# FindoraNetwork/ark-bulletproofs

Hardware: AMD Instinct MI355X
Metric: r1cs_constraints_proved_per_sec (+ r1cs_batch_verifies_per_sec under "verify") (higher is better)
Workload: dtype u32x9 (256-bit modular integers, radix 2^29)

## Files before the change

### ark_bulletproofs_amd/csrc/arkbp.hip

```cpp
#include <hip/hip_runtime.h>
#include <sys/prctl.h>
#include <time.h>
#include <rccl/rccl.h>
#include <dlfcn.h>
#include <mutex>
#include <cmath>
#include <cstdio>
#include <cstring>
#include <algorithm>
#include <deque>
#include <array>
#include <functional>
#include <map>
#include <memory>
#include <set>
#include <string>
#include <tuple>
#include <unordered_map>
#include <vector>
#include "../../include/arkbp.h"
#include <atomic>
#include <chrono>
#include "host_proto.hpp"
#include "prove_steps.hpp"
// ... 596 lines not shown
    done = !over;
    return BP_OK;
}
template <class C> static bool msm_glv_route(const bp_ctx* ctx, const BaseSegs& segs, size_t n, bool sharded, int w_hi) {
    if constexpr (!C::HAS_GLV) { (void)ctx; (void)segs; (void)n; (void)sharded; (void)w_hi; return false; }
    else {
        static const bool no_glv = getenv("ARKBP_MSM_NOGLV") != nullptr, no_fs0 = getenv("ARKBP_MSM_NOFS") != nullptr;
        return !no_glv && !no_fs0 && !sharded && w_hi < 0 && ctx->shard_world == 1 && !segs.fixed_c4 && msm_glv_sizes(msm_knobs(ctx), n);
    }
}

template <class C, class Finish>
static int msm_tree_back(bp_ctx* ctx, const BaseSegs& segs, const u32* entries, int mode, const SlotPlan& sp, const MsmPlan& pl, const u32* tot, int nl, int chl,
                         bool special, int spl, u32 b_gen, u32 top_nb, bool wave, int& K, bool& deep, Finish&& finish) {
    hipStream_t st = ctx->stream;
    const int TB = 256;
    const size_t Bp1 = (size_t)pl.B + 1;
    u32* lvl = ctx->lvl_off.as<u32>();
    K = 1;
    { u64 cap = (u64)1 << chl; while (cap < tot[MSM_NLMAX]) { cap <<= chl; K++; } }
    if (special && K < spl + 1) K = spl + 1;
    deep = K >= nl;
    if (deep) return BP_OK;
    BPCHK(ctx->lvA.ensure((size_t)tot[1] * 96));
    if (K >= 2) BPCHK(ctx->lvB.ensure((size_t)tot[2] * 96));
    if (wave && !special) {
        ScopedK acc(ctx, BP_K_MSM_ACCUM);
        hipLaunchKernelGGL(k_msm_accum_wave<C>, dim3((pl.B + 3) / 4), dim3(256), 0, st, segs, entries, lvl, lvl + Bp1 * K, ctx->lvA.as<u32>(), pl.B, mode, sp, (u32)pl.NB,
                           ctx->boff.as<u32>());
        acc.stop();
        finish(ctx->lvA.as<u32>(), lvl + Bp1 * K);
        return BP_OK;
    }
    {
        ScopedK acc(ctx, BP_K_MSM_ACCUM);
        hipLaunchKernelGGL(k_msm_accum<C>, dim3((tot[1] + TB - 1) / TB), dim3(TB), 0, st, segs, entries, lvl, lvl + Bp1, ctx->lvA.as<u32>(), pl.B, tot[1], mode, sp, (u32)pl.NB,
                           ctx->boff.as<u32>(), chl);
    }
    u32* cur = ctx->lvA.as<u32>();
    u32* nxt = ctx->lvB.as<u32>();
    ScopedK agg(ctx, BP_K_MSM_AGG);
    for (int k = 2; k <= K; k++) {
        hipLaunchKernelGGL(k_msm_reduce<C>, dim3((tot[k] + TB - 1) / TB), dim3(TB), 0, st, cur, lvl + Bp1 * (k - 1), lvl + Bp1 * k, nxt, pl.B, tot[k], chl,
                           (k == spl + 1 && special) ? b_gen : pl.B);
        if (k == spl + 1 && special)
            hipLaunchKernelGGL(k_msm_reduce_special<C>, dim3(top_nb), dim3(256), 0, st, cur, lvl + Bp1 * spl, lvl + Bp1 * (spl + 1), nxt, b_gen, pl.B);
        u32* t = cur; cur = nxt; nxt = t;
    }
    finish(cur, lvl + Bp1 * K);
    return BP_OK;
}

template <class C> static int msm_run(bp_ctx* ctx, const BaseSegs& segs, const u32* d_scalars_one, size_t n, int scalars_mont, J4& result,
                                      int w_lo = 0, int w_hi = -1 ,
                                      int shard_mode = -1 ,
                                      const ScalSegs* sseg = nullptr ,
                                      bool no_fixed_shape = false ) {
    ScalSegs d_scalars; memset(&d_scalars, 0, sizeof d_scalars);
    if (sseg) d_scalars = *sseg; else { d_scalars.nseg = 1; d_scalars.ptr[0] = d_scalars_one; d_scalars.start[0] = 0; d_scalars.start[1] = (u32)n; }
    typedef host::Grp<C> G;
    result = G::inf();
    if (n == 0) return BP_OK;
    if (n >= (1u << 31)) { g_err = "msm: n too large"; return BP_E_ARG; }
    hipStream_t st = ctx->stream;
    const MsmKnobs kn = msm_knobs(ctx);
    MsmPlan pl = msm_plan(n, C::Fr::BITS, kn);
    const bool sharded = w_hi < 0 && ctx->shard_world > 1 && shard_mode != 0;
    if (sharded && shard_mode != 2) {
        const int base = pl.W / ctx->shard_world, rem = pl.W % ctx->shard_world, r = ctx->shard_rank;
// ... 3599 lines not shown
```

### ark_bulletproofs_amd/csrc/ec.cuh

```cuda
#pragma once
#include "fp29.cuh"

namespace arkbp {

struct Aff {
    Fe x, y;
};
struct Jac {
    Fe X, Y, Z;
};

ARKBP_HD bool aff_is_inf(const Aff& p) { return fe_is_zero_exact(p.x) && fe_is_zero_exact(p.y); }
ARKBP_HD bool jac_is_inf(const Jac& p) { return fe_is_zero_exact(p.Z); }
template <class C> ARKBP_HD Jac jac_inf() {
    Jac r;
    r.X = fe_one<typename C::Fq>();
    r.Y = fe_one<typename C::Fq>();
    r.Z = fe_zero<typename C::Fq>();
    return r;
}
template <class C> ARKBP_HD Jac jac_from_aff(const Aff& p) {
    if (aff_is_inf(p)) return jac_inf<C>();
    Jac r;
    r.X = p.x;
// ... 104 lines not shown
template <class C> ARKBP_HD Jac jac_add(const Jac& p, const Jac& q) {
    typedef typename C::Fq F;
    if (jac_is_inf(q)) return p;
    if (jac_is_inf(p)) return q;
    Fe Z1Z1 = fe_sqr<F>(p.Z), Z2Z2 = fe_sqr<F>(q.Z);
    Fe U1 = fe_mul<F>(p.X, Z2Z2), U2 = fe_mul<F>(q.X, Z1Z1);
    Fe S1 = fe_mul<F>(p.Y, fe_mul<F>(q.Z, Z2Z2)), S2 = fe_mul<F>(q.Y, fe_mul<F>(p.Z, Z1Z1));
    Fe H = fe_sub<F, 2>(U2, U1);
    Fe r = fe_sub<F, 2>(S2, S1);
    if (fe_is_zero_mod<F>(H)) {
        if (fe_is_zero_mod<F>(r)) return jac_dbl<C>(p);
        return jac_inf<C>();
    }
    Fe HH = fe_sqr<F>(H);
    Fe HHH = fe_mul<F>(H, HH);
    Fe V = fe_mul<F>(U1, HH);
    Jac o;
    o.X = fe_wred<F>(fe_sub<F, 4>(fe_sqr<F>(r), fe_add(HHH, fe_dbl(V))));
    o.Y = fe_mul2<F>(r, fe_sub<F, 4>(V, o.X), fe_neg<F, 2>(S1), HHH);
    o.Z = fe_mul<F>(fe_mul<F>(p.Z, q.Z), H);
    return o;
}

template <class C> ARKBP_HD Aff jac_to_aff_with_zinv(const Jac& p, const Fe& zinv) {
    typedef typename C::Fq F;
    Aff r;
    if (jac_is_inf(p)) {
        r.x = fe_zero<F>();
        r.y = fe_zero<F>();
        return r;
    }
    Fe zi2 = fe_sqr<F>(zinv);
    r.x = fe_canon<F>(fe_mul<F>(p.X, zi2));
    r.y = fe_canon<F>(fe_mul<F>(p.Y, fe_mul<F>(zi2, zinv)));
    return r;
}
template <class C> ARKBP_HD Aff jac_to_aff(const Jac& p) {
    return jac_to_aff_with_zinv<C>(p, fe_inv<typename C::Fq>(p.Z));
}

template <class F> ARKBP_DEV_NOINLINE bool fe_sqrt(Fe& out, const Fe& a_in) {
    const Fe a = fe_wred<F>(a_in);
    if (fe_is_zero_mod<F>(a)) { out = fe_zero<F>(); return true; }
    const Fe a2 = fe_sqr<F>(a), a3 = fe_mul<F>(a2, a);
    Fe w = fe_one<F>();
#pragma unroll 1
// ... 90 lines not shown
```

### ark_bulletproofs_amd/csrc/ipa.cuh

```cuda
#pragma once
#include "msm.cuh"

namespace arkbp {

template <class F> __global__ void k_scalars_import(const u32* __restrict__ in, u32* __restrict__ out, u32 n) {
    const u32 i = blockIdx.x * blockDim.x + threadIdx.x;
    if (i >= n) return;
    u32 w[8];
    load_words8(w, in + (size_t)i * 8);
    store_fe_dev<F>(out + (size_t)i * 8, fe_load_ark<F>(w));
}
template <class F> __global__ void k_scalars_export(const u32* __restrict__ in, u32* __restrict__ out, u32 n) {
    const u32 i = blockIdx.x * blockDim.x + threadIdx.x;
    if (i >= n) return;
    u32 w[8];
    fe_store_ark<F>(w, load_fe_dev<F>(in + (size_t)i * 8));
    store_words8(out + (size_t)i * 8, w);
}

static constexpr int IMPORT_MAX = 5;
struct ImportList {
    u32* dst[IMPORT_MAX];
    u32 cnt[IMPORT_MAX];
    int nseg;
// ... 484 lines not shown
            const Aff cur = load_aff_dev(row + ((size_t)(e - 1) * n + i) * 16);
            if (!jac_equals_aff<C>(jac_madd<C>(jac_from_aff<C>(prev), base), cur)) wrong++;
            prev = cur;
        }
        expect = jac_dbl<C>(jac_from_aff<C>(prev));
    }
    if (wrong) atomicAdd(bad, (unsigned long long)wrong);
}
template <class C> __global__ void __launch_bounds__(256)
k_fb_rows_check(const u32* __restrict__ gens, const u32* __restrict__ T, u32 n, size_t row_points, u32 R, unsigned long long* __restrict__ bad) {
    const u32 i = blockIdx.x * blockDim.x + threadIdx.x;
    if (i >= n) return;
    u32 wrong = 0;
    Jac expect = jac_from_aff<C>(load_aff_dev(gens + (size_t)i * 16));
#pragma unroll 1
    for (u32 r = 0; r < R; r++) {
        const Aff cur = load_aff_dev(T + ((size_t)r * row_points + i) * 16);
        if (!jac_equals_aff<C>(expect, cur)) wrong++;
        expect = jac_dbl<C>(jac_dbl<C>(jac_dbl<C>(jac_dbl<C>(jac_from_aff<C>(cur)))));
    }
    if (wrong) atomicAdd(bad, (unsigned long long)wrong);
}

template <class C> __device__ __forceinline__ Jac ftab_step(Jac acc, const u32* __restrict__ T, u32 n_tab, u32 E, u32 gi, u32 j, u32 e1, u32 e2, bool neg1, bool neg2) {
    typedef typename C::Fq F;
#pragma unroll 1
    for (int h = 0; h < (C::HAS_GLV ? 2 : 1); h++) {
        const u32 e = h ? e2 : e1;
        if (!e) continue;
        const u32* src = T + (((size_t)j * E + (e - 1)) * n_tab + gi) * 16;
        const bool neg = h ? neg2 : neg1;
        Aff P = load_aff_dev(src);
        if constexpr (C::HAS_GLV) { if (h && !aff_is_inf(P)) P.x = fe_mul<F>(P.x, fe_const<F, C::BETA29>()); }
        bool rare;
        Jac nxt = jac_madd_fast<C>(acc, aff_cneg_lazy<C>(P, neg), rare);
        if (__builtin_expect(rare, 0)) {
            Aff Q = load_aff_dev(src);
            if constexpr (C::HAS_GLV) { if (h && !aff_is_inf(Q)) Q.x = fe_mul<F>(Q.x, fe_const<F, C::BETA29>()); }
            nxt = jac_madd<C>(acc, aff_cneg_lazy<C>(Q, neg));
        }
        acc = nxt;
    }
    return acc;
}
template <class C> __global__ void __launch_bounds__(256) __attribute__((amdgpu_waves_per_eu(3)))
k_ipa_fold_tab(const u32* __restrict__ TG, const u32* __restrict__ TH, u32 n_tab, u32 E, u32* __restrict__ G, u32* __restrict__ H, u32 n, FtabDigits dG,
               FtabDigits dH, int which, u32 g_first, u32 g_stride, u32* __restrict__ jac_ws,
               const u32* __restrict__ Gin ,
               const u32* __restrict__ Hin) {
    typedef typename C::Fq F;
    const u32 t = blockIdx.x * blockDim.x + threadIdx.x;
    if (t >= (which == 3 ? 2 * n : n)) return;
    const bool isH = which == 2 || (which == 3 && t >= n);
    const u32 i = (which == 3 && isH) ? t - n : t;
    u32* V = isH ? H : G;
    const u32* T = isH ? TH : TG;
    const u32 gi = g_first + i * g_stride;
    Jac acc = jac_inf<C>();
    const u32 nwin = isH ? dH.nwin : dG.nwin;
#pragma unroll 1
    for (u32 j = 0; j < nwin; j++) {
        const u32 e1 = isH ? dH.e1[j] : dG.e1[j], e2 = isH ? dH.e2[j] : dG.e2[j];
        acc = ftab_step<C>(acc, T, n_tab, E, gi, j, e1, e2, (((isH ? dH.neg1 : dG.neg1) >> j) & 1ull) != 0, (((isH ? dH.neg2 : dG.neg2) >> j) & 1ull) != 0);
    }
    const u32* Vin = isH ? (Hin ? Hin : H) : (Gin ? Gin : G);
    acc = jac_madd<C>(acc, load_aff_dev(Vin + (size_t)(n + i) * 16));
    fold_emit<C>(V, i, t, acc, jac_ws);
}

struct FtabDigits3 {
    FtabDigits d[3];
};
template <class C> __global__ void __launch_bounds__(256) __attribute__((amdgpu_waves_per_eu(3)))
k_ipa_fold_tab2(const u32* __restrict__ TG, const u32* __restrict__ TH, u32 n_tab, u32 E, u32* __restrict__ G, u32* __restrict__ H, u32 m, FtabDigits3 dG,
                FtabDigits3 dH, u32* __restrict__ jac_ws, const u32* __restrict__ Gin, const u32* __restrict__ Hin,
                u32 g_first , u32 g_stride) {
    typedef typename C::Fq F;
    const u32 t = blockIdx.x * blockDim.x + threadIdx.x;
    if (t >= 2 * m) return;
    const bool isH = t >= m;
    const u32 i = isH ? t - m : t;
    const u32 n = 2 * m;
    const u32* T = isH ? TH : TG;
    Jac acc = jac_inf<C>();
#pragma unroll 1
    for (u32 mu = 0; mu < 3; mu++) {
        const u32 gi = g_first + (mu == 0 ? m + i : mu == 1 ? n + i : i) * g_stride;
        const u32 nwin = isH ? dH.d[mu].nwin : dG.d[mu].nwin;
        const unsigned long long neg1 = isH ? dH.d[mu].neg1 : dG.d[mu].neg1, neg2 = isH ? dH.d[mu].neg2 : dG.d[mu].neg2;
#pragma unroll 1
        for (u32 j = 0; j < nwin; j++) {
            const u32 e1 = isH ? dH.d[mu].e1[j] : dG.d[mu].e1[j], e2 = isH ? dH.d[mu].e2[j] : dG.d[mu].e2[j];
            acc = ftab_step<C>(acc, T, n_tab, E, gi, j, e1, e2, ((neg1 >> j) & 1ull) != 0, ((neg2 >> j) & 1ull) != 0);
        }
    }
    acc = jac_madd<C>(acc, load_aff_dev((isH ? Hin : Gin) + (size_t)(n + m + i) * 16));
    fold_emit<C>(isH ? H : G, i, t, acc, jac_ws);
}

}
```

### ark_bulletproofs_amd/csrc/msm.cuh

```cuda
#pragma once
#include "ec.cuh"
#include "fe_io.cuh"
#include "ecq.cuh"
#include "glv.cuh"
#include "msm_plan.hpp"

namespace arkbp {

static constexpr int MSM_MAXSEG = 6;

struct BaseSegs {
    const u32* ptr[MSM_MAXSEG];
    u32 start[MSM_MAXSEG + 1];
    int nseg;
    u32 fixed_c4;
    u32 tbits;
    u64 row_words[MSM_MAXSEG];
    u32 glv;
    u32 stride[MSM_MAXSEG];
};
__device__ __forceinline__ const u32* seg_base_ptr(const BaseSegs& s, u32 idx) {
    u32 w = 0;
    if (s.glv) idx >>= 1;
    if (s.fixed_c4) { w = idx >> s.tbits; idx &= (1u << s.tbits) - 1u; }
// ... 34 lines not shown
    const uint4* q = reinterpret_cast<const uint4*>(p);
    Raw16 r;
    r.a = q[0]; r.b = q[1]; r.c = q[2]; r.d = q[3];
    return r;
}
__device__ __forceinline__ Aff aff_from_raw(const Raw16& r) {
    const u32 w[16] = {r.a.x, r.a.y, r.a.z, r.a.w, r.b.x, r.b.y, r.b.z, r.b.w, r.c.x, r.c.y, r.c.z, r.c.w, r.d.x, r.d.y, r.d.z, r.d.w};
    return aff_load_dev(w);
}
template <class C> __device__ __forceinline__ void store_jac_ws(u32* p, const Jac& j) {
    typedef typename C::Fq F;
    u32 w[8];
    fe_pack(w, fe_canon<F>(j.X)); store_words8(p, w);
    fe_pack(w, fe_canon<F>(j.Y)); store_words8(p + 8, w);
    fe_pack(w, fe_canon<F>(j.Z)); store_words8(p + 16, w);
}
__device__ __forceinline__ Jac load_jac_ws(const u32* p) {
    u32 w[8];
    Jac j;
    load_words8(w, p); j.X = fe_unpack(w);
    load_words8(w, p + 8); j.Y = fe_unpack(w);
    load_words8(w, p + 16); j.Z = fe_unpack(w);
    return j;
}

__device__ __forceinline__ int msm_digit(const u32 k[8], int w, int c, u32& carry) {
    const int bit = w * c;
    const int wi = bit >> 5, bo = bit & 31;
    u64 x = 0;
    if (wi < 8) x = k[wi];
    if (wi + 1 < 8) x |= (u64)k[wi + 1] << 32;
    u32 d = ((u32)(x >> bo) & ((1u << c) - 1)) + carry;
    carry = d > (1u << (c - 1)) ? 1u : 0u;
    return (int)d - (int)(carry << c);
}

__device__ __forceinline__ void load_words12(u32 w[12], const u32* p) {
    const uint4* q = reinterpret_cast<const uint4*>(p);
    const uint4 a = q[0], b = q[1], c = q[2];
    w[0] = a.x; w[1] = a.y; w[2] = a.z; w[3] = a.w; w[4] = b.x; w[5] = b.y; w[6] = b.z; w[7] = b.w; w[8] = c.x; w[9] = c.y; w[10] = c.z; w[11] = c.w;
}
__device__ __forceinline__ void store_words12(u32* p, const u32 w[12]) {
    uint4* q = reinterpret_cast<uint4*>(p);
    q[0] = make_uint4(w[0], w[1], w[2], w[3]); q[1] = make_uint4(w[4], w[5], w[6], w[7]); q[2] = make_uint4(w[8], w[9], w[10], w[11]);
}
__device__ __forceinline__ void glv_half(const u32 g[12], int h, u32 k[8], bool& neg) {
// ... 359 lines not shown
#pragma unroll
    for (int j = 0; j < 8; j++) k[j] = 0;
    if (live) load_words8(k, canon + (size_t)i * 8);
    u32 carry = 0;
    for (int w = 0; w < pl.W; w++) {
        const int d = msm_digit(k, w, pl.c, carry);
        const bool valid = live && d != 0 && w >= pl.w_lo && w < pl.w_hi;
        const u32 pos = wave_count(cursor, (u32)w * pl.NB + (u32)(d < 0 ? -d : d) - 1, valid);
        if (valid) entries[pos] = (i << 1) | (d < 0 ? 1u : 0u);
    }
}

__device__ __forceinline__ u32 find_bucket(const u32* __restrict__ off, u32 B, u32 j) {
    u32 lo = 0, hi = B;
    while (hi - lo > 1) {
        u32 mid = (lo + hi) >> 1;
        if (off[mid] <= j) lo = mid; else hi = mid;
    }
    return lo;
}

template <class C> __global__ void __launch_bounds__(256)
k_msm_accum(BaseSegs segs, const u32* __restrict__ entries, const u32* __restrict__ off0, const u32* __restrict__ off1, u32* __restrict__ out,
            u32 B, u32 nchunks, int slotted, SlotPlan sp, u32 NB, const u32* __restrict__ boff, int chl) {
    const u32 j = blockIdx.x * blockDim.x + threadIdx.x;
    if (j >= nchunks) return;
    const u32 b = find_bucket(off1, B, j);
    u32 beg, end;
    const u32 r = j - off1[b], k = off1[b + 1] - off1[b];
    u32 s0, cnt;
    if (slotted == 2) {
        s0 = boff[b]; cnt = off0[b + 1] - off0[b];
    } else if (slotted) {
        const u32 w = b / NB, v = b - w * NB;
        s0 = sp.base[w] + v * sp.cap[w]; cnt = off0[b + 1] - off0[b];
    } else {
        s0 = off0[b]; cnt = off0[b + 1] - off0[b];
    }
    const u32 per = k > 1 ? (cnt + k - 1) / k : (1u << chl);
    beg = s0 + min(r * per, cnt);
    end = min(beg + per, s0 + cnt);
    Jac acc = jac_inf<C>();
    if (beg < end) {
        u32 ent = entries[beg];
        u32 ent_n = beg + 1 < end ? entries[beg + 1] : 0u;
        Raw16 raw = load_raw16(seg_base_ptr(segs, ent >> 1));
        for (u32 e = beg; e < end; e++) {
            Raw16 raw_n = raw;
            u32 ent_nn = 0;
            if (e + 1 < end) raw_n = load_raw16(seg_base_ptr(segs, ent_n >> 1));
            if (e + 2 < end) ent_nn = entries[e + 2];
            const Aff p = aff_from_raw(raw);
            if (e == beg) {
                acc = jac_from_aff<C>(aff_cneg_lazy<C>(p, ent & 1));
                acc.Y = fe_wred<typename C::Fq>(acc.Y);
            } else {
                bool rare;
                Jac nxt = jac_madd_fast<C>(acc, aff_cneg_lazy<C>(p, ent & 1), rare);
                if (__builtin_expect(rare, 0)) nxt = jac_madd<C>(acc, aff_cneg_lazy<C>(load_aff_dev(seg_base_ptr(segs, ent >> 1)), ent & 1));
                acc = nxt;
            }
            ent = ent_n; ent_n = ent_nn;
            raw = raw_n;
        }
    }
    store_jac_ws<C>(out + (size_t)j * 24, acc);
}

template <class C> __global__ void __launch_bounds__(256)
k_msm_accum_wave(BaseSegs segs, const u32* __restrict__ entries, const u32* __restrict__ off0, const u32* __restrict__ off_last, u32* __restrict__ out, u32 B,
                 int slotted, SlotPlan sp, u32 NB, const u32* __restrict__ boff) {
    __shared__ u32 sh[4][64 * 27];
    const u32 wv = threadIdx.x >> 6, lane = threadIdx.x & 63;
    const u32 b = blockIdx.x * 4 + wv;
    if (b >= B) return;
    const u32 cnt = off0[b + 1] - off0[b];
    if (!cnt) return;
    u32 beg;
    if (slotted == 2) beg = boff[b];
    else if (slotted) { const u32 w = b / NB, v = b - w * NB; beg = sp.base[w] + v * sp.cap[w]; }
    else beg = off0[b];
    Jac acc = jac_inf<C>();
    for (u32 e = lane; e < cnt; e += 64) {
        const u32 ent = entries[beg + e];
        acc = jac_madd<C>(acc, aff_cneg_lazy<C>(load_aff_dev(seg_base_ptr(segs, ent >> 1)), ent & 1));
    }
    u32* s = sh[wv];
    for (u32 stride = 32; stride >= 1; stride >>= 1) {
        if (lane >= stride && lane < 2 * stride) {
#pragma unroll
            for (int i = 0; i < 9; i++) { s[i * 64 + lane] = acc.X.l[i]; s[(9 + i) * 64 + lane] = acc.Y.l[i]; s[(18 + i) * 64 + lane] = acc.Z.l[i]; }
        }
        __builtin_amdgcn_wave_barrier();
        __threadfence_block();
        if (lane < stride) {
            Jac o;
#pragma unroll
            for (int i = 0; i < 9; i++) { o.X.l[i] = s[i * 64 + lane + stride]; o.Y.l[i] = s[(9 + i) * 64 + lane + stride]; o.Z.l[i] = s[(18 + i) * 64 + lane + stride]; }
            acc = jac_add<C>(acc, o);
        }
        __builtin_amdgcn_wave_barrier();
        __threadfence_block();
    }
    if (lane == 0) store_jac_ws<C>(out + (size_t)off_last[b] * 24, acc);
}

template <class C> __global__ void __launch_bounds__(256)
k_msm_reduce(const u32* __restrict__ in, const u32* __restrict__ off_prev, const u32* __restrict__ off_cur, u32* __restrict__ out, u32 B,
             u32 nchunks, int chl, u32 skip_from ) {
    const u32 j = blockIdx.x * blockDim.x + threadIdx.x;
    if (j >= nchunks) return;
    const u32 b = find_bucket(off_cur, B, j);
    if (b >= skip_from) return;
    const u32 beg = off_prev[b] + ((j - off_cur[b]) << chl);
    const u32 end = min(beg + (1u << chl), off_prev[b + 1]);
    Jac acc = load_jac_ws(in + (size_t)beg * 24);
    for (u32 e = beg + 1; e < end; e++) acc = jac_add<C>(acc, load_jac_ws(in + (size_t)e * 24));
    store_jac_ws<C>(out + (size_t)j * 24, acc);
}

template <class C, u32 NT = 256> __device__ __forceinline__ Jac block_sum_jac(Jac acc, u32* __restrict__ sh ) {
    const u32 tid = threadIdx.x;
    for (u32 stride = NT / 2; stride >= 1; stride >>= 1) {
        if (tid >= stride && tid < 2 * stride) {
#pragma unroll
            for (int i = 0; i < 9; i++) { sh[i * NT + tid] = acc.X.l[i]; sh[(9 + i) * NT + tid] = acc.Y.l[i]; sh[(18 + i) * NT + tid] = acc.Z.l[i]; }
        }
        __syncthreads();
        if (tid < stride) {
            Jac o;
#pragma unroll
            for (int i = 0; i < 9; i++) { o.X.l[i] = sh[i * NT + tid + stride]; o.Y.l[i] = sh[(9 + i) * NT + tid + stride]; o.Z.l[i] = sh[(18 + i) * NT + tid + stride]; }
            acc = jac_add<C>(acc, o);
        }
        __syncthreads();
    }
    return acc;
}
// ... 8 lines not shown
    return o;
}
template <class C, u32 NT = 256> __device__ __forceinline__ Jac block_sum_jac_quad(const Jac& acc, u32* __restrict__ sh ) {
    const u32 tid = threadIdx.x, q = tid & 3u, quad = tid >> 2;
    lds_put_jac(sh, NT, tid, acc);
    __syncthreads();
#pragma unroll 1
    for (u32 half = NT / 2; half >= 1; half >>= 1) {
#pragma unroll 1
        for (u32 j = quad; j < half; j += NT / 4) {
            const Jac r = qjac_add<C>(lds_get_jac(sh, NT, j), lds_get_jac(sh, NT, j + half), q);
            if (q == 0) lds_put_jac(sh, NT, j, r);
        }
        __syncthreads();
    }
    return lds_get_jac(sh, NT, 0);
}
__device__ __forceinline__ Jac jac_shfl_down(const Jac& a, int o, int width = 64) {
    Jac r;
#pragma unroll
    for (int i = 0; i < 9; i++) { r.X.l[i] = __shfl_down(a.X.l[i], o, width); r.Y.l[i] = __shfl_down(a.Y.l[i], o, width); r.Z.l[i] = __shfl_down(a.Z.l[i], o, width); }
    return r;
}
template <class C> __global__ void __launch_bounds__(256)
k_msm_reduce_special(const u32* __restrict__ in, const u32* __restrict__ off1, const u32* __restrict__ off2, u32* __restrict__ out, u32 b_gen, u32 B) {
    __shared__ u32 sh[256 * 27];
    const u32 b = b_gen + blockIdx.x;
    if (b >= B) return;
    const u32 beg = off1[b], end = off1[b + 1];
    if (beg == end) return;
    Jac acc = jac_inf<C>();
    for (u32 e = beg + threadIdx.x; e < end; e += 256) acc = jac_add<C>(acc, load_jac_ws(in + (size_t)e * 24));
    acc = block_sum_jac<C>(acc, sh);
    if (threadIdx.x == 0) store_jac_ws<C>(out + (size_t)off2[b] * 24, acc);
}

template <class C> __global__ void __launch_bounds__(256)
k_msm_marginals(const u32* __restrict__ sums, const u32* __restrict__ off, u32* __restrict__ T_out, MsmPlan pl) {
    typedef typename C::Fq F;
    __shared__ u32 sh[256 * 27];
    const int w = blockIdx.x, k = blockIdx.y;
    const u32 tid = threadIdx.x;
    Jac acc = jac_inf<C>();
    for (u32 idx = tid; idx < (u32)pl.NB; idx += 256) {
        if (!(((idx + 1) >> k) & 1)) continue;
        const u32 b = (u32)w * pl.NB + idx;
        const u32 o = off[b];
        if (off[b + 1] == o) continue;
        acc = jac_add<C>(acc, load_jac_ws(sums + (size_t)o * 24));
    }
    acc = block_sum_jac<C>(acc, sh);
    if (tid == 0) {
        u32* o = T_out + ((size_t)w * pl.c + k) * 24;
        u32 wd[8];
        const bool inf = jac_is_inf(acc);
// ... 182 lines not shown
    const u32 job = blockIdx.z;
    const BaseSegs& segs = bjobs.j[job];
    entries += job * jb.slots; bcnt += job * jb.buckets; loff += job * jb.buckets; boff += job * jb.buckets; bin_chunks += job * jb.binch;
    out += job * jb.part; info += job * jb.T;
    fs_block_scan(bin_chunks, fp.nbins, base, ws);
    const u32 total = min(base[fp.nbins], fp.max_chunks);
    if (blockIdx.x == 0 && threadIdx.x == 0) { info[0] = base[fp.nbins]; info[1] = base[fp.nbins - 1]; }
    const u32 j = blockIdx.x * 256u + threadIdx.x;
    if (j >= total) return;
    u32 lo = 0, hi = fp.nbins;
    while (hi - lo > 1) { const u32 mid = (lo + hi) >> 1; if (base[mid] <= j) lo = mid; else hi = mid; }
    const u32 jj = j - base[lo];
    u32 b0, nb;
    fs_bin_range(lo, pl, bp, b0, nb);
    u32 l2 = 0, h2 = nb;
    while (h2 - l2 > 1) { const u32 mid = (l2 + h2) >> 1; if (loff[b0 + mid] <= jj) l2 = mid; else h2 = mid; }
    const u32 b = b0 + l2;
    const u32 s0 = boff[b];
    const u32 cnt = bcnt[b], r = jj - loff[b];
    const u32 k = (cnt + chcap - 1u) / chcap;
    const u32 per = k > 1 ? (cnt + k - 1) / k : chcap;
    const u32 beg = s0 + min(r * per, cnt);
    const u32 end = min(beg + per, s0 + cnt);
    Jac acc = jac_inf<C>();
    if (beg < end) {
        u32 ent = entries[beg];
        u32 ent_n = beg + 1 < end ? entries[beg + 1] : 0u;
        Raw16 raw = load_raw16(seg_base_ptr(segs, ent >> 1));
        for (u32 e = beg; e < end; e++) {
            Raw16 raw_n = raw;
            u32 ent_nn = 0;
            if (e + 1 < end) raw_n = load_raw16(seg_base_ptr(segs, ent_n >> 1));
            if (e + 2 < end) ent_nn = entries[e + 2];
            Aff p = aff_from_raw(raw);
            if constexpr (C::HAS_GLV) {
                if (segs.glv && (ent & 2u) && !aff_is_inf(p)) p.x = fe_mul<typename C::Fq>(p.x, fe_const<typename C::Fq, C::BETA29>());
            }
            if (e == beg) {
                acc = jac_from_aff<C>(aff_cneg_lazy<C>(p, ent & 1));
                acc.Y = fe_wred<typename C::Fq>(acc.Y);
            } else {
                bool rare;
                Jac nxt = jac_madd_fast<C>(acc, aff_cneg_lazy<C>(p, ent & 1), rare);
                if (__builtin_expect(rare, 0)) {
                    Aff q = load_aff_dev(seg_base_ptr(segs, ent >> 1));
                    if constexpr (C::HAS_GLV) {
                        if (segs.glv && (ent & 2u) && !aff_is_inf(q)) q.x = fe_mul<typename C::Fq>(q.x, fe_const<typename C::Fq, C::BETA29>());
                    }
                    nxt = jac_madd<C>(acc, aff_cneg_lazy<C>(q, ent & 1));
                }
                acc = nxt;
            }
            ent = ent_n; ent_n = ent_nn;
            raw = raw_n;
        }
    }
    store_jac_ws<C>(out + (size_t)j * 24, acc);
}
template <class C, bool QUAD = false> __global__ void __launch_bounds__(256)
k_msm_reduce_fs(const u32* __restrict__ part, const u32* __restrict__ bcnt, const u32* __restrict__ loff, const u32* __restrict__ bin_chunks,
                u32* __restrict__ sums, MsmPlan pl, BinPlan bp, FsPlan fp, u32 chcap, u32 G, FsJobs jb) {
    __shared__ u32 base[MSM_FS_MAXBINS + 1];
    __shared__ u32 ws[4];
    const u32 job = blockIdx.z;
    part += job * jb.part; bcnt += job * jb.buckets; loff += job * jb.buckets; bin_chunks += job * jb.binch; sums += job * jb.sums;
    fs_block_scan(bin_chunks, fp.nbins, base, ws);
    const u32 g = blockIdx.x * 256u + threadIdx.x;
    const u32 nbk = bp.wb * (u32)pl.NB;
    const u32 gb = G == 4 ? g >> 2 : g;
    const u32 b = min(gb, nbk - 1u), q = G == 4 ? g & 3u : 0u;
    const u32 w = b / (u32)pl.NB, v = b - w * (u32)pl.NB;
    const u32 first = base[w * bp.NBIN + (v >> bp.LB)] + loff[b];
    u32 nch = min((bcnt[b] + chcap - 1u) / chcap, MSM_FS_BUCKET_MAX / 8u);
    if (first + nch > fp.max_chunks) nch = 0;
    if (QUAD) {
        Jac acc = jac_inf<C>();
        if (nch) acc = load_jac_ws(part + (size_t)first * 24);
#pragma unroll 1
        for (u32 e = 1; e < nch; e++) acc = qjac_add<C>(acc, load_jac_ws(part + (size_t)(first + e) * 24), q);
        if (q == 0 && gb < nbk) store_jac_ws<C>(sums + (size_t)b * 24, acc);
// ... 208 lines not shown
```

Baseline: 17.69 million.

## Accumulate MSM buckets and fixed-table folds in XYZZ coordinates

```diff
diff --git a/ark_bulletproofs_amd/csrc/arkbp.hip b/ark_bulletproofs_amd/csrc/arkbp.hip
--- a/ark_bulletproofs_amd/csrc/arkbp.hip
+++ b/ark_bulletproofs_amd/csrc/arkbp.hip
@@ -642,7 +642,8 @@
     if (special && K < spl + 1) K = spl + 1;
     deep = K >= nl;
     if (deep) return BP_OK;
-    BPCHK(ctx->lvA.ensure((size_t)tot[1] * 96));
+    const bool xl1 = K >= 2 && !(wave && !special);
+    BPCHK(ctx->lvA.ensure((size_t)tot[1] * (xl1 ? MSM_XYZZ_WORDS * 4 : 96)));
     if (K >= 2) BPCHK(ctx->lvB.ensure((size_t)tot[2] * 96));
     if (wave && !special) {
         ScopedK acc(ctx, BP_K_MSM_ACCUM);
@@ -655,16 +656,20 @@
     {
         ScopedK acc(ctx, BP_K_MSM_ACCUM);
         hipLaunchKernelGGL(k_msm_accum<C>, dim3((tot[1] + TB - 1) / TB), dim3(TB), 0, st, segs, entries, lvl, lvl + Bp1, ctx->lvA.as<u32>(), pl.B, tot[1], mode, sp, (u32)pl.NB,
-                           ctx->boff.as<u32>(), chl);
+                           ctx->boff.as<u32>(), chl, xl1 ? 1 : 0);
     }
     u32* cur = ctx->lvA.as<u32>();
     u32* nxt = ctx->lvB.as<u32>();
     ScopedK agg(ctx, BP_K_MSM_AGG);
     for (int k = 2; k <= K; k++) {
-        hipLaunchKernelGGL(k_msm_reduce<C>, dim3((tot[k] + TB - 1) / TB), dim3(TB), 0, st, cur, lvl + Bp1 * (k - 1), lvl + Bp1 * k, nxt, pl.B, tot[k], chl,
-                           (k == spl + 1 && special) ? b_gen : pl.B);
-        if (k == spl + 1 && special)
-            hipLaunchKernelGGL(k_msm_reduce_special<C>, dim3(top_nb), dim3(256), 0, st, cur, lvl + Bp1 * spl, lvl + Bp1 * (spl + 1), nxt, b_gen, pl.B);
+        const dim3 rg((tot[k] + TB - 1) / TB);
+        const u32 skip = (k == spl + 1 && special) ? b_gen : pl.B;
+        if (k == 2) hipLaunchKernelGGL((k_msm_reduce<C, true>), rg, dim3(TB), 0, st, cur, lvl + Bp1 * (k - 1), lvl + Bp1 * k, nxt, pl.B, tot[k], chl, skip);
+        else hipLaunchKernelGGL((k_msm_reduce<C, false>), rg, dim3(TB), 0, st, cur, lvl + Bp1 * (k - 1), lvl + Bp1 * k, nxt, pl.B, tot[k], chl, skip);
+        if (k == spl + 1 && special) {
+            if (spl == 1) hipLaunchKernelGGL((k_msm_reduce_special<C, true>), dim3(top_nb), dim3(256), 0, st, cur, lvl + Bp1 * spl, lvl + Bp1 * (spl + 1), nxt, b_gen, pl.B);
+            else hipLaunchKernelGGL((k_msm_reduce_special<C, false>), dim3(top_nb), dim3(256), 0, st, cur, lvl + Bp1 * spl, lvl + Bp1 * (spl + 1), nxt, b_gen, pl.B);
+        }
         u32* t = cur; cur = nxt; nxt = t;
     }
     finish(cur, lvl + Bp1 * K);
diff --git a/ark_bulletproofs_amd/csrc/ec.cuh b/ark_bulletproofs_amd/csrc/ec.cuh
--- a/ark_bulletproofs_amd/csrc/ec.cuh
+++ b/ark_bulletproofs_amd/csrc/ec.cuh
@@ -150,6 +150,90 @@
     return o;
 }
 
+struct Xyzz {
+    Fe X, Y, ZZ, ZZZ;
+};
+ARKBP_HD bool xyzz_is_inf(const Xyzz& p) { return fe_is_zero_exact(p.ZZ); }
+template <class C> ARKBP_HD Xyzz xyzz_inf() {
+    Xyzz r;
+    r.X = fe_one<typename C::Fq>();
+    r.Y = fe_one<typename C::Fq>();
+    r.ZZ = fe_zero<typename C::Fq>();
+    r.ZZZ = fe_zero<typename C::Fq>();
+    return r;
+}
+template <class C> ARKBP_HD Xyzz xyzz_from_aff(const Aff& q) {
+    typedef typename C::Fq F;
+    if (aff_is_inf(q)) return xyzz_inf<C>();
+    Xyzz r;
+    r.X = q.x;
+    r.Y = fe_wred<F>(q.y);
+    r.ZZ = fe_one<F>();
+    r.ZZZ = fe_one<F>();
+    return r;
+}
+template <class C> ARKBP_HD Xyzz jac_to_xyzz(const Jac& p) {
+    typedef typename C::Fq F;
+    Xyzz r;
+    r.X = p.X;
+    r.Y = p.Y;
+    r.ZZ = fe_sqr<F>(p.Z);
+    r.ZZZ = fe_mul<F>(p.Z, r.ZZ);
+    return r;
+}
+template <class C> ARKBP_HD Jac xyzz_to_jac(const Xyzz& p) {
+    typedef typename C::Fq F;
+    const Fe z4 = fe_sqr<F>(p.ZZ);
+    Jac r;
+    r.X = fe_mul<F>(p.X, z4);
+    r.Y = fe_mul<F>(p.Y, fe_mul<F>(z4, p.ZZ));
+    r.Z = xyzz_is_inf(p) ? fe_zero<F>() : p.ZZZ;
+    return r;
+}
+
+template <class C> ARKBP_HD Xyzz xyzz_madd_fast(const Xyzz& p, const Aff& q, bool& rare) {
+    typedef typename C::Fq F;
+    Fe U2 = fe_mul<F>(q.x, p.ZZ);
+    Fe S2 = fe_mul<F>(q.y, p.ZZZ);
+    Fe P = fe_sub<F, 4>(U2, p.X);
+    Fe R = fe_sub<F, 4>(S2, p.Y);
+    rare = aff_is_inf(q) | xyzz_is_inf(p) | fe_maybe_zero_mod<F>(P);
+    Fe PP = fe_sqr<F>(P);
+    Fe PPP = fe_mul<F>(P, PP);
+    Fe Q = fe_mul<F>(p.X, PP);
+    Xyzz o;
+    o.X = fe_wred<F>(fe_sub<F, 4>(fe_sqr<F>(R), fe_add(PPP, fe_dbl(Q))));
+    o.Y = fe_mul2<F>(R, fe_sub<F, 4>(Q, o.X), fe_neg<F, 4>(p.Y), PPP);
+    o.ZZ = fe_mul<F>(p.ZZ, PP);
+    o.ZZZ = fe_mul<F>(p.ZZZ, PPP);
+    return o;
+}
+template <class C> ARKBP_HD Xyzz xyzz_madd(const Xyzz& p, const Aff& q) {
+    return jac_to_xyzz<C>(jac_madd<C>(xyzz_to_jac<C>(p), q));
+}
+template <class C> ARKBP_HD Xyzz xyzz_add(const Xyzz& p, const Xyzz& q) {
+    typedef typename C::Fq F;
+    if (xyzz_is_inf(q)) return p;
+    if (xyzz_is_inf(p)) return q;
+    Fe U1 = fe_mul<F>(p.X, q.ZZ), U2 = fe_mul<F>(q.X, p.ZZ);
+    Fe S1 = fe_mul<F>(p.Y, q.ZZZ), S2 = fe_mul<F>(q.Y, p.ZZZ);
+    Fe P = fe_sub<F, 2>(U2, U1);
+    Fe R = fe_sub<F, 2>(S2, S1);
+    if (fe_is_zero_mod<F>(P)) {
+        if (fe_is_zero_mod<F>(R)) return jac_to_xyzz<C>(jac_dbl<C>(xyzz_to_jac<C>(p)));
+        return xyzz_inf<C>();
+    }
+    Fe PP = fe_sqr<F>(P);
+    Fe PPP = fe_mul<F>(P, PP);
+    Fe Q = fe_mul<F>(U1, PP);
+    Xyzz o;
+    o.X = fe_wred<F>(fe_sub<F, 4>(fe_sqr<F>(R), fe_add(PPP, fe_dbl(Q))));
+    o.Y = fe_mul2<F>(R, fe_sub<F, 4>(Q, o.X), fe_neg<F, 2>(S1), PPP);
+    o.ZZ = fe_mul<F>(fe_mul<F>(p.ZZ, q.ZZ), PP);
+    o.ZZZ = fe_mul<F>(fe_mul<F>(p.ZZZ, q.ZZZ), PPP);
+    return o;
+}
+
 template <class C> ARKBP_HD Aff jac_to_aff_with_zinv(const Jac& p, const Fe& zinv) {
     typedef typename C::Fq F;
     Aff r;
diff --git a/ark_bulletproofs_amd/csrc/ipa.cuh b/ark_bulletproofs_amd/csrc/ipa.cuh
--- a/ark_bulletproofs_amd/csrc/ipa.cuh
+++ b/ark_bulletproofs_amd/csrc/ipa.cuh
@@ -530,7 +530,7 @@
     if (wrong) atomicAdd(bad, (unsigned long long)wrong);
 }
 
-template <class C> __device__ __forceinline__ Jac ftab_step(Jac acc, const u32* __restrict__ T, u32 n_tab, u32 E, u32 gi, u32 j, u32 e1, u32 e2, bool neg1, bool neg2) {
+template <class C> __device__ __forceinline__ Xyzz ftab_step(Xyzz acc, const u32* __restrict__ T, u32 n_tab, u32 E, u32 gi, u32 j, u32 e1, u32 e2, bool neg1, bool neg2) {
     typedef typename C::Fq F;
 #pragma unroll 1
     for (int h = 0; h < (C::HAS_GLV ? 2 : 1); h++) {
@@ -541,15 +541,21 @@
         Aff P = load_aff_dev(src);
         if constexpr (C::HAS_GLV) { if (h && !aff_is_inf(P)) P.x = fe_mul<F>(P.x, fe_const<F, C::BETA29>()); }
         bool rare;
-        Jac nxt = jac_madd_fast<C>(acc, aff_cneg_lazy<C>(P, neg), rare);
+        Xyzz nxt = xyzz_madd_fast<C>(acc, aff_cneg_lazy<C>(P, neg), rare);
         if (__builtin_expect(rare, 0)) {
             Aff Q = load_aff_dev(src);
             if constexpr (C::HAS_GLV) { if (h && !aff_is_inf(Q)) Q.x = fe_mul<F>(Q.x, fe_const<F, C::BETA29>()); }
-            nxt = jac_madd<C>(acc, aff_cneg_lazy<C>(Q, neg));
+            nxt = xyzz_madd<C>(acc, aff_cneg_lazy<C>(Q, neg));
         }
         acc = nxt;
     }
     return acc;
+}
+template <class C> __device__ __forceinline__ Jac ftab_close(const Xyzz& acc, const u32* __restrict__ src) {
+    bool rare;
+    Xyzz nxt = xyzz_madd_fast<C>(acc, load_aff_dev(src), rare);
+    if (__builtin_expect(rare, 0)) nxt = xyzz_madd<C>(acc, load_aff_dev(src));
+    return xyzz_to_jac<C>(nxt);
 }
 template <class C> __global__ void __launch_bounds__(256) __attribute__((amdgpu_waves_per_eu(3)))
 k_ipa_fold_tab(const u32* __restrict__ TG, const u32* __restrict__ TH, u32 n_tab, u32 E, u32* __restrict__ G, u32* __restrict__ H, u32 n, FtabDigits dG,
@@ -564,7 +570,7 @@
     u32* V = isH ? H : G;
     const u32* T = isH ? TH : TG;
     const u32 gi = g_first + i * g_stride;
-    Jac acc = jac_inf<C>();
+    Xyzz acc = xyzz_inf<C>();
     const u32 nwin = isH ? dH.nwin : dG.nwin;
 #pragma unroll 1
     for (u32 j = 0; j < nwin; j++) {
@@ -572,8 +578,7 @@
         acc = ftab_step<C>(acc, T, n_tab, E, gi, j, e1, e2, (((isH ? dH.neg1 : dG.neg1) >> j) & 1ull) != 0, (((isH ? dH.neg2 : dG.neg2) >> j) & 1ull) != 0);
     }
     const u32* Vin = isH ? (Hin ? Hin : H) : (Gin ? Gin : G);
-    acc = jac_madd<C>(acc, load_aff_dev(Vin + (size_t)(n + i) * 16));
-    fold_emit<C>(V, i, t, acc, jac_ws);
+    fold_emit<C>(V, i, t, ftab_close<C>(acc, Vin + (size_t)(n + i) * 16), jac_ws);
 }
 
 struct FtabDigits3 {
@@ -590,7 +595,7 @@
     const u32 i = isH ? t - m : t;
     const u32 n = 2 * m;
     const u32* T = isH ? TH : TG;
-    Jac acc = jac_inf<C>();
+    Xyzz acc = xyzz_inf<C>();
 #pragma unroll 1
     for (u32 mu = 0; mu < 3; mu++) {
         const u32 gi = g_first + (mu == 0 ? m + i : mu == 1 ? n + i : i) * g_stride;
@@ -602,8 +607,7 @@
             acc = ftab_step<C>(acc, T, n_tab, E, gi, j, e1, e2, ((neg1 >> j) & 1ull) != 0, ((neg2 >> j) & 1ull) != 0);
         }
     }
-    acc = jac_madd<C>(acc, load_aff_dev((isH ? Hin : Gin) + (size_t)(n + m + i) * 16));
-    fold_emit<C>(isH ? H : G, i, t, acc, jac_ws);
-}
-
-}
+    fold_emit<C>(isH ? H : G, i, t, ftab_close<C>(acc, (isH ? Hin : Gin) + (size_t)(n + m + i) * 16), jac_ws);
+}
+
+}
diff --git a/ark_bulletproofs_amd/csrc/msm.cuh b/ark_bulletproofs_amd/csrc/msm.cuh
--- a/ark_bulletproofs_amd/csrc/msm.cuh
+++ b/ark_bulletproofs_amd/csrc/msm.cuh
@@ -80,6 +80,24 @@
     load_words8(w, p + 8); j.Y = fe_unpack(w);
     load_words8(w, p + 16); j.Z = fe_unpack(w);
     return j;
+}
+static constexpr u32 MSM_XYZZ_WORDS = 32;
+template <class C> __device__ __forceinline__ void store_xyzz_ws(u32* p, const Xyzz& a) {
+    typedef typename C::Fq F;
+    u32 w[8];
+    fe_pack(w, fe_canon<F>(a.X)); store_words8(p, w);
+    fe_pack(w, fe_canon<F>(a.Y)); store_words8(p + 8, w);
+    fe_pack(w, fe_canon<F>(a.ZZ)); store_words8(p + 16, w);
+    fe_pack(w, fe_canon<F>(a.ZZZ)); store_words8(p + 24, w);
+}
+__device__ __forceinline__ Xyzz load_xyzz_ws(const u32* p) {
+    u32 w[8];
+    Xyzz a;
+    load_words8(w, p); a.X = fe_unpack(w);
+    load_words8(w, p + 8); a.Y = fe_unpack(w);
+    load_words8(w, p + 16); a.ZZ = fe_unpack(w);
+    load_words8(w, p + 24); a.ZZZ = fe_unpack(w);
+    return a;
 }
 
 __device__ __forceinline__ int msm_digit(const u32 k[8], int w, int c, u32& carry) {
@@ -485,7 +503,8 @@
 
 template <class C> __global__ void __launch_bounds__(256)
 k_msm_accum(BaseSegs segs, const u32* __restrict__ entries, const u32* __restrict__ off0, const u32* __restrict__ off1, u32* __restrict__ out,
-            u32 B, u32 nchunks, int slotted, SlotPlan sp, u32 NB, const u32* __restrict__ boff, int chl) {
+            u32 B, u32 nchunks, int slotted, SlotPlan sp, u32 NB, const u32* __restrict__ boff, int chl,
+            int xyzz_out ) {
     const u32 j = blockIdx.x * blockDim.x + threadIdx.x;
     if (j >= nchunks) return;
     const u32 b = find_bucket(off1, B, j);
@@ -503,7 +522,7 @@
     const u32 per = k > 1 ? (cnt + k - 1) / k : (1u << chl);
     beg = s0 + min(r * per, cnt);
     end = min(beg + per, s0 + cnt);
-    Jac acc = jac_inf<C>();
+    Xyzz acc = xyzz_inf<C>();
     if (beg < end) {
         u32 ent = entries[beg];
         u32 ent_n = beg + 1 < end ? entries[beg + 1] : 0u;
@@ -515,19 +534,19 @@
             if (e + 2 < end) ent_nn = entries[e + 2];
             const Aff p = aff_from_raw(raw);
             if (e == beg) {
-                acc = jac_from_aff<C>(aff_cneg_lazy<C>(p, ent & 1));
-                acc.Y = fe_wred<typename C::Fq>(acc.Y);
+                acc = xyzz_from_aff<C>(aff_cneg_lazy<C>(p, ent & 1));
             } else {
                 bool rare;
-                Jac nxt = jac_madd_fast<C>(acc, aff_cneg_lazy<C>(p, ent & 1), rare);
-                if (__builtin_expect(rare, 0)) nxt = jac_madd<C>(acc, aff_cneg_lazy<C>(load_aff_dev(seg_base_ptr(segs, ent >> 1)), ent & 1));
+                Xyzz nxt = xyzz_madd_fast<C>(acc, aff_cneg_lazy<C>(p, ent & 1), rare);
+                if (__builtin_expect(rare, 0)) nxt = xyzz_madd<C>(acc, aff_cneg_lazy<C>(load_aff_dev(seg_base_ptr(segs, ent >> 1)), ent & 1));
                 acc = nxt;
             }
             ent = ent_n; ent_n = ent_nn;
             raw = raw_n;
         }
     }
-    store_jac_ws<C>(out + (size_t)j * 24, acc);
+    if (xyzz_out) store_xyzz_ws<C>(out + (size_t)j * MSM_XYZZ_WORDS, acc);
+    else store_jac_ws<C>(out + (size_t)j * 24, xyzz_to_jac<C>(acc));
 }
 
 template <class C> __global__ void __launch_bounds__(256)
@@ -568,7 +587,7 @@
     if (lane == 0) store_jac_ws<C>(out + (size_t)off_last[b] * 24, acc);
 }
 
-template <class C> __global__ void __launch_bounds__(256)
+template <class C, bool XIN = false> __global__ void __launch_bounds__(256)
 k_msm_reduce(const u32* __restrict__ in, const u32* __restrict__ off_prev, const u32* __restrict__ off_cur, u32* __restrict__ out, u32 B,
              u32 nchunks, int chl, u32 skip_from ) {
     const u32 j = blockIdx.x * blockDim.x + threadIdx.x;
@@ -577,6 +596,12 @@
     if (b >= skip_from) return;
     const u32 beg = off_prev[b] + ((j - off_cur[b]) << chl);
     const u32 end = min(beg + (1u << chl), off_prev[b + 1]);
+    if constexpr (XIN) {
+        Xyzz xacc = load_xyzz_ws(in + (size_t)beg * MSM_XYZZ_WORDS);
+        for (u32 e = beg + 1; e < end; e++) xacc = xyzz_add<C>(xacc, load_xyzz_ws(in + (size_t)e * MSM_XYZZ_WORDS));
+        store_jac_ws<C>(out + (size_t)j * 24, xyzz_to_jac<C>(xacc));
+        return;
+    }
     Jac acc = load_jac_ws(in + (size_t)beg * 24);
     for (u32 e = beg + 1; e < end; e++) acc = jac_add<C>(acc, load_jac_ws(in + (size_t)e * 24));
     store_jac_ws<C>(out + (size_t)j * 24, acc);
@@ -631,7 +656,7 @@
     for (int i = 0; i < 9; i++) { r.X.l[i] = __shfl_down(a.X.l[i], o, width); r.Y.l[i] = __shfl_down(a.Y.l[i], o, width); r.Z.l[i] = __shfl_down(a.Z.l[i], o, width); }
     return r;
 }
-template <class C> __global__ void __launch_bounds__(256)
+template <class C, bool XIN = false> __global__ void __launch_bounds__(256)
 k_msm_reduce_special(const u32* __restrict__ in, const u32* __restrict__ off1, const u32* __restrict__ off2, u32* __restrict__ out, u32 b_gen, u32 B) {
     __shared__ u32 sh[256 * 27];
     const u32 b = b_gen + blockIdx.x;
@@ -639,7 +664,13 @@
     const u32 beg = off1[b], end = off1[b + 1];
     if (beg == end) return;
     Jac acc = jac_inf<C>();
-    for (u32 e = beg + threadIdx.x; e < end; e += 256) acc = jac_add<C>(acc, load_jac_ws(in + (size_t)e * 24));
+    if constexpr (XIN) {
+        Xyzz xacc = xyzz_inf<C>();
+        for (u32 e = beg + threadIdx.x; e < end; e += 256) xacc = xyzz_add<C>(xacc, load_xyzz_ws(in + (size_t)e * MSM_XYZZ_WORDS));
+        acc = xyzz_to_jac<C>(xacc);
+    } else {
+        for (u32 e = beg + threadIdx.x; e < end; e += 256) acc = jac_add<C>(acc, load_jac_ws(in + (size_t)e * 24));
+    }
     acc = block_sum_jac<C>(acc, sh);
     if (threadIdx.x == 0) store_jac_ws<C>(out + (size_t)off2[b] * 24, acc);
 }
@@ -868,7 +899,7 @@
     const u32 per = k > 1 ? (cnt + k - 1) / k : chcap;
     const u32 beg = s0 + min(r * per, cnt);
     const u32 end = min(beg + per, s0 + cnt);
-    Jac acc = jac_inf<C>();
+    Xyzz acc = xyzz_inf<C>();
     if (beg < end) {
         u32 ent = entries[beg];
         u32 ent_n = beg + 1 < end ? entries[beg + 1] : 0u;
@@ -883,17 +914,16 @@
                 if (segs.glv && (ent & 2u) && !aff_is_inf(p)) p.x = fe_mul<typename C::Fq>(p.x, fe_const<typename C::Fq, C::BETA29>());
             }
             if (e == beg) {
-                acc = jac_from_aff<C>(aff_cneg_lazy<C>(p, ent & 1));
-                acc.Y = fe_wred<typename C::Fq>(acc.Y);
+                acc = xyzz_from_aff<C>(aff_cneg_lazy<C>(p, ent & 1));
             } else {
                 bool rare;
-                Jac nxt = jac_madd_fast<C>(acc, aff_cneg_lazy<C>(p, ent & 1), rare);
+                Xyzz nxt = xyzz_madd_fast<C>(acc, aff_cneg_lazy<C>(p, ent & 1), rare);
                 if (__builtin_expect(rare, 0)) {
                     Aff q = load_aff_dev(seg_base_ptr(segs, ent >> 1));
                     if constexpr (C::HAS_GLV) {
                         if (segs.glv && (ent & 2u) && !aff_is_inf(q)) q.x = fe_mul<typename C::Fq>(q.x, fe_const<typename C::Fq, C::BETA29>());
                     }
-                    nxt = jac_madd<C>(acc, aff_cneg_lazy<C>(q, ent & 1));
+                    nxt = xyzz_madd<C>(acc, aff_cneg_lazy<C>(q, ent & 1));
                 }
                 acc = nxt;
             }
@@ -901,7 +931,7 @@
             raw = raw_n;
         }
     }
-    store_jac_ws<C>(out + (size_t)j * 24, acc);
+    store_jac_ws<C>(out + (size_t)j * 24, xyzz_to_jac<C>(acc));
 }
 template <class C, bool QUAD = false> __global__ void __launch_bounds__(256)
 k_msm_reduce_fs(const u32* __restrict__ part, const u32* __restrict__ bcnt, const u32* __restrict__ loff, const u32* __restrict__ bin_chunks,
diff --git a/ark_bulletproofs_amd/csrc/xyzz_selftest.cpp b/ark_bulletproofs_amd/csrc/xyzz_selftest.cpp
--- /dev/null
+++ b/ark_bulletproofs_amd/csrc/xyzz_selftest.cpp
@@ -0,0 +1,186 @@
+#include <cstdio>
+#include <cstdlib>
+#include <cstring>
+#include <vector>
+#include "ec.cuh"
+#include "host_math.hpp"
+using namespace arkbp;
+using host::A4;
+using host::F4;
+using host::J4;
+
+static int g_fail = 0;
+#define CHECK(c, ...) do { if (!(c)) { if (g_fail < 20) { fprintf(stderr, "FAIL %s:%d: ", __FILE__, __LINE__); fprintf(stderr, __VA_ARGS__); fprintf(stderr, "\n"); } g_fail++; } } while (0)
+
+static uint64_t g_rng = 0x9e3779b97f4a7c15ull;
+static uint64_t rnd() {
+    uint64_t z = (g_rng += 0x9e3779b97f4a7c15ull);
+    z = (z ^ (z >> 30)) * 0xbf58476d1ce4e5b9ull;
+    z = (z ^ (z >> 27)) * 0x94d049bb133111ebull;
+    return z ^ (z >> 31);
+}
+
+template <class C> struct T {
+    typedef typename C::Fq F;
+    typedef host::Grp<C> G;
+    typedef host::Fld<F> HF;
+
+    static Aff dev(const A4& a) { u32 w[16]; memcpy(w, a.x.v, 32); memcpy(w + 8, a.y.v, 32); return aff_load_ark<C>(w); }
+    static Fe dev_fe(const F4& a) { u32 w[8]; memcpy(w, a.v, 32); return fe_load_ark<F>(w); }
+    static A4 host_of(const Jac& j) { u32 w[16]; A4 o; aff_store_ark<C>(w, jac_to_aff<C>(j)); memcpy(o.x.v, w, 32); memcpy(o.y.v, w + 8, 32); return o; }
+    static A4 host_of(const Xyzz& p) { return host_of(xyzz_to_jac<C>(p)); }
+    static A4 hadd(const A4& a, const A4& b) { return G::to_aff(G::add(G::from_aff(a), G::from_aff(b))); }
+    static A4 hneg(const A4& a) { return a.is_inf() ? a : G::neg(a); }
+    static A4 random_point() {
+        uint64_t k[4] = {rnd(), rnd(), rnd(), rnd() >> 2};
+        return G::to_aff(G::mul_canon(G::generator(), k));
+    }
+    static Xyzz madd_hot(const Xyzz& acc, const Aff& q, bool* was_rare = nullptr) {
+        bool rare;
+        Xyzz nxt = xyzz_madd_fast<C>(acc, q, rare);
+        if (rare) nxt = xyzz_madd<C>(acc, q);
+        if (was_rare) *was_rare = rare;
+        return nxt;
+    }
+    static Aff neg_lazy(const Aff& p, bool at_bound) {
+        Aff r = aff_cneg_lazy<C>(p, true);
+        if (at_bound && !aff_is_inf(p)) r.y = fe_norm(fe_add(r.y, fe_const<F, F::P29>()));
+        return r;
+    }
+    static Xyzz blurred(const A4& a, const A4& b) {
+        Xyzz acc = xyzz_from_aff<C>(dev(a));
+        acc = madd_hot(acc, dev(b));
+        return madd_hot(acc, neg_lazy(dev(b), false));
+    }
+
+    static void random_ops(const std::vector<A4>& pool, int rounds) {
+        const size_t n = pool.size();
+        for (int it = 0; it < rounds; it++) {
+            const A4 &a = pool[rnd() % n], &b = pool[rnd() % n], &c = pool[rnd() % n], &d = pool[rnd() % n];
+            const A4 ab = hadd(a, b), cd = hadd(c, d);
+            Xyzz acc = madd_hot(xyzz_from_aff<C>(dev(a)), dev(b));
+            CHECK(host_of(acc) == ab, "madd_hot, round %d", it);
+            CHECK(host_of(madd_hot(acc, dev(c))) == hadd(ab, c), "madd_hot on a general accumulator, round %d", it);
+            CHECK(host_of(xyzz_madd<C>(acc, dev(c))) == hadd(ab, c), "xyzz_madd, round %d", it);
+            CHECK(host_of(madd_hot(acc, neg_lazy(dev(c), it & 1))) == hadd(ab, hneg(c)), "madd_hot with a lazy negation, round %d", it);
+            const Xyzz acc2 = madd_hot(xyzz_from_aff<C>(dev(c)), dev(d));
+            CHECK(host_of(xyzz_add<C>(acc, acc2)) == hadd(ab, cd), "xyzz_add, round %d", it);
+            const Jac j = xyzz_to_jac<C>(acc);
+            CHECK(host_of(j) == ab, "xyzz_to_jac, round %d", it);
+            const Jac j2 = jac_dbl<C>(j);
+            CHECK(host_of(jac_to_xyzz<C>(j2)) == hadd(ab, ab), "jac_to_xyzz, round %d", it);
+            CHECK(host_of(jac_add<C>(xyzz_to_jac<C>(jac_to_xyzz<C>(j2)), j)) == hadd(hadd(ab, ab), ab), "round trip, round %d", it);
+        }
+    }
+
+    static void chains(const std::vector<A4>& pool, int count) {
+        const size_t n = pool.size();
+        for (int ch = 0; ch < count; ch++) {
+            A4 want = pool[rnd() % n];
+            Xyzz acc = xyzz_from_aff<C>(dev(want));
+            Xyzz other = xyzz_from_aff<C>(dev(pool[rnd() % n]));
+            A4 want_other = host_of(other);
+            for (int s = 0; s < 64; s++) {
+                const A4& q = pool[rnd() % n];
+                const bool neg = s & 1;
+                acc = madd_hot(acc, neg ? neg_lazy(dev(q), (s & 2) != 0) : dev(q));
+                want = hadd(want, neg ? hneg(q) : q);
+                CHECK(host_of(acc) == want, "chain %d step %d", ch, s);
+                if ((s & 7) == 7) {
+                    other = xyzz_add<C>(other, acc);
+                    want_other = hadd(want_other, want);
+                    CHECK(host_of(other) == want_other, "chain %d step %d: xyzz_add", ch, s);
+                }
+            }
+        }
+    }
+
+    static void exceptions(const std::vector<A4>& pool) {
+        const A4 inf = G::aff_inf();
+        for (size_t i = 0; i + 1 < pool.size() && i < 24; i++) {
+            const A4 &a = pool[i], &b = pool[i + 1];
+            const Xyzz A = blurred(a, b), A1 = xyzz_from_aff<C>(dev(a)), I = xyzz_inf<C>();
+            const A4 aa = hadd(a, a);
+            bool rare;
+            CHECK(host_of(madd_hot(A, dev(a), &rare)) == aa && rare, "P + P (hot)");
+            CHECK(host_of(madd_hot(A1, dev(a), &rare)) == aa && rare, "P + P (hot, lifted)");
+            CHECK(host_of(xyzz_madd<C>(A, dev(a))) == aa, "P + P (xyzz_madd)");
+            CHECK(host_of(xyzz_add<C>(A, A1)) == aa && host_of(xyzz_add<C>(A1, A)) == aa && host_of(xyzz_add<C>(A, A)) == aa, "P + P (xyzz_add)");
+            for (int bound = 0; bound < 2; bound++) {
+                const Xyzz r = madd_hot(A, neg_lazy(dev(a), bound), &rare);
+                CHECK(xyzz_is_inf(r) && rare && host_of(r) == inf, "P - P (hot)");
+                CHECK(xyzz_is_inf(xyzz_madd<C>(A, neg_lazy(dev(a), bound))), "P - P (xyzz_madd)");
+            }
+            const Xyzz NA = blurred(hneg(a), b);
+            CHECK(xyzz_is_inf(xyzz_add<C>(A, NA)) && xyzz_is_inf(xyzz_add<C>(NA, A1)), "P - P (xyzz_add)");
+            CHECK(host_of(madd_hot(A, dev(inf), &rare)) == a && rare, "P + 0 (hot)");
+            CHECK(host_of(madd_hot(I, dev(a), &rare)) == a && rare, "0 + P (hot)");
+            CHECK(host_of(madd_hot(I, neg_lazy(dev(a), true), &rare)) == hneg(a) && rare, "0 - P (hot)");
+            CHECK(xyzz_is_inf(madd_hot(I, dev(inf), &rare)) && rare, "0 + 0 (hot)");
+            CHECK(host_of(xyzz_madd<C>(A, dev(inf))) == a && host_of(xyzz_madd<C>(I, dev(a))) == a && xyzz_is_inf(xyzz_madd<C>(I, dev(inf))), "identity (xyzz_madd)");
+            CHECK(host_of(xyzz_add<C>(A, I)) == a && host_of(xyzz_add<C>(I, A)) == a && xyzz_is_inf(xyzz_add<C>(I, I)), "identity (xyzz_add)");
+            CHECK(xyzz_is_inf(xyzz_from_aff<C>(dev(inf))) && jac_is_inf(xyzz_to_jac<C>(I)) && xyzz_is_inf(jac_to_xyzz<C>(jac_inf<C>())), "identity (conversions)");
+            Xyzz acc = A1;
+            acc = madd_hot(acc, dev(b));
+            acc = madd_hot(acc, neg_lazy(dev(b), true));
+            acc = madd_hot(acc, neg_lazy(dev(a), false), &rare);
+            CHECK(xyzz_is_inf(acc) && rare, "chain through the identity: the sum is not the identity");
+            acc = madd_hot(acc, dev(b), &rare);
+            CHECK(rare && host_of(acc) == b, "chain through the identity: the lift after it");
+            acc = madd_hot(acc, dev(a));
+            acc = madd_hot(acc, dev(a));
+            CHECK(host_of(acc) == hadd(hadd(b, a), a), "chain through the identity: the additions after it");
+        }
+    }
+
+    static void low_limb_collision(const std::vector<A4>& pool) {
+        F4 two232 = HF::from_u64(1ull << 58);
+        two232 = HF::sqr(HF::sqr(two232));
+        const F4 inv232 = HF::inv(two232);
+        int done = 0;
+        for (size_t i = 0; i + 1 < pool.size() && done < 8; i++) {
+            const A4 &a = pool[i], &q = pool[i + 1];
+            const F4 d = HF::sub(q.x, a.x);
+            if (d.is_zero()) continue;
+            const F4 dinv = HF::inv(d);
+            for (uint64_t j = 1; j < 64; j++) {
+                const F4 l2 = HF::mul(HF::mul(HF::from_u64(j), inv232), dinv);
+                F4 l;
+                if (!HF::sqrt(l, l2)) continue;
+                const F4 l3 = HF::mul(l2, l);
+                Xyzz acc;
+                acc.X = dev_fe(HF::mul(a.x, l2));
+                acc.Y = dev_fe(HF::mul(a.y, l3));
+                acc.ZZ = dev_fe(l2);
+                acc.ZZZ = dev_fe(l3);
+                CHECK(host_of(acc) == a, "scaled representative");
+                bool rare;
+                const Xyzz fast = xyzz_madd_fast<C>(acc, dev(q), rare);
+                CHECK(rare, "low-limb collision (j = %llu): the filter did not fire", (unsigned long long)j);
+                CHECK(host_of(fast) == hadd(a, q), "low-limb collision: the one-block result itself (P != 0, so it is a valid sum)");
+                CHECK(host_of(madd_hot(acc, dev(q))) == hadd(a, q), "low-limb collision: the redo");
+                done++;
+                break;
+            }
+        }
+        CHECK(done == 8, "low-limb collision: only %d cases built", done);
+    }
+
+    static void run(const char* name) {
+        std::vector<A4> pool;
+        for (int i = 0; i < 48; i++) pool.push_back(random_point());
+        random_ops(pool, 3000);
+        chains(pool, 24);
+        exceptions(pool);
+        low_limb_collision(pool);
+        printf("%s: %s\n", name, g_fail ? "FAILED" : "ok");
+    }
+};
+
+int main() {
+    T<Secq>::run("secq256k1");
+    T<Zorro>::run("zorro");
+    if (g_fail) { printf("xyzz selftest: %d failures\n", g_fail); return 1; }
+    printf("xyzz selftest ok\n");
+    return 0;
+}
```

Result: no change. 17.66 million (-0.2%).
